# rahulaggarwal965/vslam

Hardware: AMD Instinct MI355X
Metric: frame-pairs/sec (extract+match+RANSAC) @1280×720, 2k kp, 4096 hyp; 1/2/4/8 GPU (higher is better)
Workload: dtype u8/f32/f64; 1 GPU; C3: 1280x720, 2000 keypoints, 4096 hypotheses, batch 256 pairs per GPU, SURVEY 8(d) data: rotation + parallax, sub-pixel resampling, 40-45 % outlier matches; pairs_per_gpu=256, batches_in_flight=4

## Files before the change

### vslam_amd/csrc/ransac_count.hip

```cpp
#include "ransac_residual.h"

namespace {
using namespace vs_ransac;

constexpr int kCntHyps = 128;
constexpr int kCntWaves = 8;
constexpr int kCntQueue = 320;
constexpr int kCntLdsMatches = 4096;
constexpr int kScreenMatches = 128;
constexpr int kScreenHyps = 128;
constexpr int kRankThreads = 512;
constexpr int kPilotHyps = kRankThreads / 64;
constexpr int kCandMax = 8;
constexpr float kCntTinyDD = 0x1p-120f;
constexpr int kFcmpOGT = 2, kFcmpOLT = 4, kFcmpULT = 12;
constexpr int kCntRec = 12;
typedef __attribute__((address_space(3))) volatile uint32_t cnt_queue_t;
static_assert(VSLAM_MAX_KP <= 65536, "queue words keep the match index in 16 bits");

__host__ __device__ constexpr int cnt_pad(int n) { return (n + 255) & ~255; }

struct CntBand {
    float lo, hi;
    double beta;
    bool ok;
};
__device__ __forceinline__ CntBand cnt_band(const float *f, float C1, float C2, float threshold) {
    CntBand B;
    bool ok = threshold >= 0x1p-20f && threshold <= 0x1p20f && C1 <= 0x1p20f && C2 <= 0x1p20f;
#pragma unroll
    for (int k = 0; k < 9; k++) ok = ok && fabsf(f[k]) <= 1024.f;
    const double S = ((double)fabsf(f[0]) + (double)fabsf(f[3]) + (double)fabsf(f[1]) + (double)fabsf(f[4])) * (double)C2 +
                     (double)fabsf(f[6]) + (double)fabsf(f[7]);
    const double beta = 4.04 * 0x1p-24 * S + 1e-30;
    const double sq = sqrt((double)threshold);
    const double lo_r = sq * (1.0 - 0x1p-20) - 1.01 * beta;
    const double hi_r = sq * (1.0 + 0x1p-20) + 2.5 * beta;
    B.lo = lo_r > 0 ? (float)(lo_r * lo_r * (1.0 - 0x1p-22)) : -1.f;
    B.hi = (float)(hi_r * hi_r * (1.0 + 0x1p-20) * (1.0 + 0x1p-22));
    if (!ok) {
        B.lo = -1.f;
        B.hi = INFINITY;
    }
    B.beta = beta;
    B.ok = ok;
    return B;
}
__device__ __forceinline__ void cnt_store_record(float *d, const float *f, const CntBand &B) {
#pragma unroll
    for (int k = 0; k < 9; k++) d[k] = f[k];
    d[9] = B.lo;
    d[10] = B.hi;
    d[11] = B.ok ? (float)(B.beta * (1.0 + 0x1p-20)) : -1.f;
}

struct CntRec {
    float f[9];
    float lo, hi;
    float beta;
};
__device__ __forceinline__ void cnt_load_record(CntRec &R, const float *s_rec, int hh) {
    const float4 *r4 = reinterpret_cast<const float4 *>(s_rec + hh * kCntRec);
    const float4 v0 = r4[0], v1 = r4[1], v2 = r4[2];
    const float f[9] = {v0.x, v0.y, v0.z, v0.w, v1.x, v1.y, v1.z, v1.w, v2.x};
#pragma unroll
    for (int k = 0; k < 9; k++) R.f[k] = f[k];
    R.lo = v2.y;
    R.hi = v2.z;
    R.beta = v2.w;
}

__device__ __forceinline__ v2f cnt_splat(float f) {
    v2f r;
    r.x = f;
    r.y = f;
    return r;
}
__device__ __forceinline__ v2f cnt_cheap(const CntRec &R, const v2f X1, const v2f Y1, const v2f X2, const v2f Y2, v2f &dd) {
    const v2f f0 = cnt_splat(R.f[0]), f1 = cnt_splat(R.f[1]), f2 = cnt_splat(R.f[2]), f3 = cnt_splat(R.f[3]), f4 = cnt_splat(R.f[4]),
              f5 = cnt_splat(R.f[5]), f6 = cnt_splat(R.f[6]), f7 = cnt_splat(R.f[7]), f8 = cnt_splat(R.f[8]);
    const v2f a0 = (f0 * X1 + f1 * Y1) + f2;
    const v2f a1 = (f3 * X1 + f4 * Y1) + f5;
    const v2f a2 = (f6 * X1 + f7 * Y1) + f8;
    const v2f n = (X2 * a0 + Y2 * a1) + a2;
    const v2f nn = n * n;
    dd = a0 * a0;
    v2f r;
    r.x = __builtin_amdgcn_rcpf(dd.x);
    r.y = __builtin_amdgcn_rcpf(dd.y);
    v2f g = __builtin_elementwise_fma(a1, a1, nn * r);
    const v2f t0 = __builtin_elementwise_fma(f3, Y2, __builtin_elementwise_fma(f0, X2, f6));
    const v2f t1 = __builtin_elementwise_fma(f4, Y2, __builtin_elementwise_fma(f1, X2, f7));
    g = __builtin_elementwise_fma(t0, t0, g);
    g = __builtin_elementwise_fma(t1, t1, g);
    return g;
}

__device__ __forceinline__ void cnt_drain(const cnt_queue_t *q, int from, int count, int lane, const float *s_rec,
                                          int *s_cnt, const float *cx1, const float *cy1, const float *cx2, const float *cy2,
                                          float threshold) {
    if (lane < count) {
        const uint32_t en = q[from + lane];
        const int hh = (int)(en >> 16), i = (int)(en & 0xFFFFu);
        ResidualF R;
#pragma unroll
        for (int k = 0; k < 9; k++) R.f[k] = s_rec[hh * kCntRec + k];
        residual_prepare(R);
        const float x2 = cx2[i], y2 = cy2[i];
        const float e = residual_e(R, make_float4(cx1[i], cy1[i], x2, y2), (double)x2, (double)y2);
        if (e <= threshold) atomicAdd(&s_cnt[hh], 1);
    }
}

__device__ __forceinline__ void cnt_push(cnt_queue_t *q, int &qn, unsigned long long U, int hh, int idx, int lane) {
    const int rank = (int)__builtin_amdgcn_mbcnt_hi((uint32_t)(U >> 32), __builtin_amdgcn_mbcnt_lo((uint32_t)U, 0u));
    if ((U >> lane) & 1ull) q[qn + rank] = ((uint32_t)hh << 16) | (uint32_t)idx;
    qn += __popcll(U);
}

template <bool PARTIAL>
__device__ __forceinline__ void cnt_eval_pair(const CntRec &R, const v2f X1, const v2f Y1, const v2f X2, const v2f Y2, int ix,
                                              int m, int &cnt, unsigned long long &ua, unsigned long long &ub,
                                              float &ddmin, v2f &acc) {
    v2f dd;
    v2f g = cnt_cheap(R, X1, Y1, X2, Y2, dd);
    ddmin = fminf(ddmin, fminf(dd.x, dd.y));
    unsigned long long ia = __builtin_amdgcn_fcmpf(g.x, R.lo, kFcmpOLT), oa = __builtin_amdgcn_fcmpf(g.x, R.hi, kFcmpOGT);
    unsigned long long ib = __builtin_amdgcn_fcmpf(g.y, R.lo, kFcmpOLT), ob = __builtin_amdgcn_fcmpf(g.y, R.hi, kFcmpOGT);
    if (PARTIAL) {
        const bool in_a = ix < m, in_b = ix + 1 < m;
        const unsigned long long va = __ballot(in_a), vb = __ballot(in_b);
        ia &= va;
        ib &= vb;
        ua = va & ~(ia | oa);
        ub = vb & ~(ib | ob);
        g.x = in_a ? g.x : 0.f;
        g.y = in_b ? g.y : 0.f;
    } else {
        ua = ~(ia | oa);
        ub = ~(ib | ob);
    }
    cnt += __popcll(ia) + __popcll(ib);
    acc += g;
}

__device__ __forceinline__ float wave_sum_to_lane63(float v) {
    const int z = 0;
    v += __int_as_float(__builtin_amdgcn_update_dpp(z, __float_as_int(v), 0xB1, 0xF, 0xF, false));
    v += __int_as_float(__builtin_amdgcn_update_dpp(z, __float_as_int(v), 0x4E, 0xF, 0xF, false));
    v += __int_as_float(__builtin_amdgcn_update_dpp(z, __float_as_int(v), 0x141, 0xF, 0xF, false));
    v += __int_as_float(__builtin_amdgcn_update_dpp(z, __float_as_int(v), 0x140, 0xF, 0xF, false));
    v += __int_as_float(__builtin_amdgcn_update_dpp(z, __float_as_int(v), 0x142, 0xA, 0xF, false));
    v += __int_as_float(__builtin_amdgcn_update_dpp(z, __float_as_int(v), 0x143, 0xC, 0xF, false));
    return v;
}

template <bool PARTIAL>
__device__ __forceinline__ void cnt_sub_block(const CntRec &R, const float4 X1, const float4 Y1, const float4 X2, const float4 Y2,
                                              int ix, int hh, int lane, int m, int &cnt, cnt_queue_t *q, int &qn, v2f &acc,
                                              int *s_unk, int &pot, bool &unk) {
    unsigned long long u0, u1, u2, u3;
    int c = 0;
    float ddmin = INFINITY;
    v2f x1a, y1a, x2a, y2a, x1b, y1b, x2b, y2b;
    x1a.x = X1.x; x1a.y = X1.y; x1b.x = X1.z; x1b.y = X1.w;
    y1a.x = Y1.x; y1a.y = Y1.y; y1b.x = Y1.z; y1b.y = Y1.w;
    x2a.x = X2.x; x2a.y = X2.y; x2b.x = X2.z; x2b.y = X2.w;
    y2a.x = Y2.x; y2a.y = Y2.y; y2b.x = Y2.z; y2b.y = Y2.w;
    cnt_eval_pair<PARTIAL>(R, x1a, y1a, x2a, y2a, ix, m, c, u0, u1, ddmin, acc);
    cnt_eval_pair<PARTIAL>(R, x1b, y1b, x2b, y2b, ix + 2, m, c, u2, u3, ddmin, acc);
    if (__builtin_amdgcn_fcmpf(ddmin, kCntTinyDD, kFcmpULT) != 0ull) {
        if (lane == 0) s_unk[hh] = 1;
        unk = true;
        c = 0;
        u0 = __builtin_amdgcn_sicmp(ix, m, 40);
        u1 = __builtin_amdgcn_sicmp(ix + 1, m, 40);
        u2 = __builtin_amdgcn_sicmp(ix + 2, m, 40);
        u3 = __builtin_amdgcn_sicmp(ix + 3, m, 40);
    }
    cnt += c;
    pot += c;
    if ((u0 | u1 | u2 | u3) != 0ull) {
        pot += __popcll(u0) + __popcll(u1) + __popcll(u2) + __popcll(u3);
        if (u0) cnt_push(q, qn, u0, hh, ix, lane);
        if (u1) cnt_push(q, qn, u1, hh, ix + 1, lane);
        if (u2) cnt_push(q, qn, u2, hh, ix + 2, lane);
        if (u3) cnt_push(q, qn, u3, hh, ix + 3, lane);
    }
}

__device__ __forceinline__ int cnt_exact_ranked(const float *F9, const float *r, int kp_pad, int m, float threshold, int lane,
                                                double *sum_out = nullptr) {
    ResidualF R;
#pragma unroll
    for (int j = 0; j < 9; j++) R.f[j] = F9[j];
    residual_prepare(R);
    int count = 0;
    double esum = 0;
    for (int i0 = 0; i0 < m; i0 += 256) {
        float4 c[4];
#pragma unroll
        for (int u = 0; u < 4; u++) {
            const int i = i0 + u * 64 + lane;
            c[u] = make_float4(r[i], r[kp_pad + i], r[2 * kp_pad + i], r[3 * kp_pad + i]);
        }
#pragma unroll
        for (int u = 0; u < 4; u++) {
            const float e = residual_e(R, c[u], (double)c[u].z, (double)c[u].w);
            count += __popcll(__ballot(i0 + u * 64 + lane < m && e <= threshold));
            if (sum_out && i0 + u * 64 + lane < m) esum += (double)e;
        }
    }
    if (sum_out) {
#pragma unroll
        for (int off = 32; off > 0; off >>= 1) esum += __shfl_xor(esum, off, 64);
        *sum_out = esum;
    }
    return count;
}

__global__ __launch_bounds__(kRankThreads) void ransac_rank_kernel(
    const float *__restrict__ xy1, const float *__restrict__ xy2, const int32_t *__restrict__ pairs,
    const int32_t *__restrict__ m_arr, int min_m, int kp_stride, int kp_pad, int hyp, float threshold,
    const float *__restrict__ hypF, int32_t *__restrict__ cbound, float *__restrict__ rk, float *__restrict__ cmax,
    unsigned long long *__restrict__ sfloor) {
    const int b = blockIdx.x, tid = threadIdx.x, lane = tid & 63;
    const int wave = __builtin_amdgcn_readfirstlane(tid >> 6);
    const int m = min(m_arr[b], kp_stride);
    if (m < min_m) return;
    __shared__ double s_psum[kPilotHyps];
    __shared__ unsigned long long s_bits[kPilotHyps][VSLAM_MAX_KP / 64];
    __shared__ int s_hist[kPilotHyps][kPilotHyps + 1], s_off[kPilotHyps][kPilotHyps + 1], s_pcount[kPilotHyps];
    const float2 *P1 = reinterpret_cast<const float2 *>(xy1) + (size_t)b * kp_stride;
    const float2 *P2 = reinterpret_cast<const float2 *>(xy2) + (size_t)b * kp_stride;
    const int2 *PR = reinterpret_cast<const int2 *>(pairs) + (size_t)b * kp_stride;
    const int npil = min(kPilotHyps, hyp);
    const int G = (m + 63) >> 6;

    if (wave < npil) {
        const int h = (int)(((long long)hyp * wave) / npil);
        ResidualF R;
        const float *src = hypF + ((size_t)b * hyp + h) * 9;
#pragma unroll
        for (int j = 0; j < 9; j++) R.f[j] = src[j];
        residual_prepare(R);
        int count = 0;
        double esum = 0;
        float c1 = 0.f, c2 = 0.f;
        for (int g0 = 0; g0 < G; g0 += 4) {
            int2 pr[4];
            float2 a[4], c[4];
#pragma unroll
            for (int u = 0; u < 4; u++) pr[u] = PR[min((g0 + u) * 64 + lane, m - 1)];
#pragma unroll
            for (int u = 0; u < 4; u++) {
                a[u] = P1[pr[u].x];
                c[u] = P2[pr[u].y];
            }
#pragma unroll
            for (int u = 0; u < 4; u++) {
                const float e = residual_e(R, make_float4(a[u].x, a[u].y, c[u].x, c[u].y), (double)c[u].x, (double)c[u].y);
                const unsigned long long in = __ballot((g0 + u) * 64 + lane < m && e <= threshold);
                count += __popcll(in);
                if ((g0 + u) * 64 + lane < m) esum += (double)e;
                if (lane == 0 && g0 + u < G) s_bits[wave][g0 + u] = in;
                c1 = fmaxf(c1, fmaxf(fabsf(a[u].x), fabsf(a[u].y)));
                c2 = fmaxf(c2, fmaxf(fabsf(c[u].x), fabsf(c[u].y)));
            }
        }
#pragma unroll
        for (int off = 32; off > 0; off >>= 1) esum += __shfl_xor(esum, off, 64);
        if (lane == 0) {
            s_pcount[wave] = count;
            s_psum[wave] = esum;
        }
        if (wave == 0) {
#pragma unroll
            for (int off = 32; off > 0; off >>= 1) {
                c1 = fmaxf(c1, __shfl_xor(c1, off, 64));
                c2 = fmaxf(c2, __shfl_xor(c2, off, 64));
            }
            if (lane == 0) {
                cmax[2 * b] = c1;
                cmax[2 * b + 1] = c2;
            }
        }
    }
    __syncthreads();

    const int gpw = (G + kPilotHyps - 1) / kPilotHyps;
    const int g_lo = min(G, wave * gpw), g_hi = min(G, g_lo + gpw);
    int hist[kPilotHyps + 1];
#pragma unroll
    for (int v = 0; v <= kPilotHyps; v++) hist[v] = 0;
    for (int g = g_lo; g < g_hi; g++) {
        const bool valid = g * 64 + lane < m;
        int key = 0;
        for (int w = 0; w < npil; w++) key += (int)((~s_bits[w][g] >> lane) & 1ull);
#pragma unroll
        for (int v = 0; v <= kPilotHyps; v++) hist[v] += __popcll(__ballot(valid && key == v));
    }
    if (lane == 0) {
#pragma unroll
        for (int v = 0; v <= kPilotHyps; v++) s_hist[wave][v] = hist[v];
    }
    __syncthreads();
    if (tid == 0) {
        int best = 0;
        for (int w = 0; w < npil; w++) best = max(best, s_pcount[w]);
        cbound[b] = best;
        if (sfloor) {
            double fl = -INFINITY;
            bool any_nan = false;
            for (int w = 0; w < npil; w++)
                if (s_pcount[w] == best) {
                    any_nan = any_nan || !(s_psum[w] == s_psum[w]);
                    if (s_psum[w] > fl) fl = s_psum[w];
                }
            const bool valid = best > 0 && !any_nan && fl > 0 && fl < 0x1p120;
            sfloor[b] = valid ? ((unsigned long long)(uint32_t)best << 32) | (unsigned long long)__float_as_uint((float)(fl * (1.0 - 0x1p-20))) : 0ull;
        }
        int run = 0;
        for (int v = kPilotHyps; v >= 0; v--)
            for (int w = 0; w < kPilotHyps; w++) {
                s_off[w][v] = run;
                run += s_hist[w][v];
            }
    }
    __syncthreads();
    int off[kPilotHyps + 1];
#pragma unroll
    for (int v = 0; v <= kPilotHyps; v++) off[v] = s_off[wave][v];
    float *r = rk + (size_t)b * 4 * kp_pad;
    for (int g = g_lo; g < g_hi; g++) {
        const int i = g * 64 + lane;
        const bool valid = i < m;
        int key = 0;
        for (int w = 0; w < npil; w++) key += (int)((~s_bits[w][g] >> lane) & 1ull);
        int pos = 0;
#pragma unroll
        for (int v = 0; v <= kPilotHyps; v++) {
            const unsigned long long bal = __ballot(valid && key == v);
            const int rank = (int)__builtin_amdgcn_mbcnt_hi((uint32_t)(bal >> 32), __builtin_amdgcn_mbcnt_lo((uint32_t)bal, 0u));
            if (key == v) pos = off[v] + rank;
            off[v] += __popcll(bal);
        }
        if (valid) {
            const int2 pr = PR[i];
            const float2 a = P1[pr.x], c = P2[pr.y];
            r[pos] = a.x;
            r[kp_pad + pos] = a.y;
            r[2 * kp_pad + pos] = c.x;
            r[3 * kp_pad + pos] = c.y;
        }
    }
    const int mpad = cnt_pad(m);
    if (m + tid < mpad) {
        const int2 pr = PR[m - 1];
        const float2 a = P1[pr.x], c = P2[pr.y];
        r[m + tid] = a.x;
        r[kp_pad + m + tid] = a.y;
        r[2 * kp_pad + m + tid] = c.x;
        r[3 * kp_pad + m + tid] = c.y;
    }
}

__global__ __launch_bounds__(256) void ransac_screen_kernel(
    const float *__restrict__ rk, int kp_pad, const int32_t *__restrict__ m_arr, int min_m, int kp_stride, int hyp,
    float threshold, const float *__restrict__ hypF, const float *__restrict__ cmax, int32_t *__restrict__ pot0) {
    const int b = blockIdx.y, tid = threadIdx.x, lane = tid & 63;
    const int wave = __builtin_amdgcn_readfirstlane(tid >> 6);
    const int hbase = blockIdx.x * kScreenHyps;
    const int m = min(m_arr[b], kp_stride);
    if (m < min_m) return;
    __shared__ __align__(16) float s_rec[kScreenHyps * kCntRec];
    if (tid < kScreenHyps) {
        const float *src = hypF + ((size_t)b * hyp + min(hbase + tid, hyp - 1)) * 9;
        float f[9];
#pragma unroll
        for (int k = 0; k < 9; k++) f[k] = src[k];
        const CntBand B = cnt_band(f, cmax[2 * b], cmax[2 * b + 1], threshold);
        cnt_store_record(s_rec + tid * kCntRec, f, B);
    }
    const int n0 = min(m, kScreenMatches);
    const float *r = rk + (size_t)b * 4 * kp_pad;
    const float2 x1 = *reinterpret_cast<const float2 *>(r + 2 * lane);
    const float2 y1 = *reinterpret_cast<const float2 *>(r + kp_pad + 2 * lane);
    const float2 x2 = *reinterpret_cast<const float2 *>(r + 2 * kp_pad + 2 * lane);
    const float2 y2 = *reinterpret_cast<const float2 *>(r + 3 * kp_pad + 2 * lane);
    v2f X1, Y1, X2, Y2;
    X1.x = x1.x; X1.y = x1.y; Y1.x = y1.x; Y1.y = y1.y;
    X2.x = x2.x; X2.y = x2.y; Y2.x = y2.x; Y2.y = y2.y;
    const unsigned long long va = __ballot(2 * lane < n0), vb = __ballot(2 * lane + 1 < n0);
    __syncthreads();
    int mine = 0;
    constexpr int kU = 4;
    for (int j = 0; j < 32; j += kU) {
        CntRec R[kU];
        v2f dd[kU], g[kU];
#pragma unroll
        for (int u = 0; u < kU; u++) cnt_load_record(R[u], s_rec, wave * 32 + j + u);
#pragma unroll
        for (int u = 0; u < kU; u++) g[u] = cnt_cheap(R[u], X1, Y1, X2, Y2, dd[u]);
#pragma unroll
        for (int u = 0; u < kU; u++) {
            const unsigned long long oa = __builtin_amdgcn_fcmpf(g[u].x, R[u].hi, kFcmpOGT), ob = __builtin_amdgcn_fcmpf(g[u].y, R[u].hi, kFcmpOGT);
            int p = __popcll(va & ~oa) + __popcll(vb & ~ob);
            if (__builtin_amdgcn_fcmpf(fminf(dd[u].x, dd[u].y), kCntTinyDD, kFcmpULT) != 0ull) p = n0;
            mine = lane == j + u ? p : mine;
        }
    }
    const int h = hbase + wave * 32 + lane;
    if (lane < 32 && h < hyp) pot0[(size_t)b * hyp + h] = mine;
}

__global__ __launch_bounds__(64 * kCandMax) void ransac_cand_kernel(
    const float *__restrict__ rk, int kp_pad, const int32_t *__restrict__ m_arr, int min_m, int kp_stride, int hyp,
    float threshold, const float *__restrict__ hypF, const int32_t *__restrict__ pot0, int by_sum,
    int32_t *__restrict__ cbound, unsigned long long *__restrict__ sfloor) {
    const int b = blockIdx.x, tid = threadIdx.x, lane = tid & 63;
    const int wave = __builtin_amdgcn_readfirstlane(tid >> 6);
    const int m = min(m_arr[b], kp_stride);
    if (m < min_m) return;
    __shared__ int s_max[kCandMax], s_l0[kCandMax][kCandMax], s_l1[kCandMax][kCandMax], s_n0[kCandMax], s_n1[kCandMax];
    __shared__ int s_cand[kCandMax], s_nc;
    const int32_t *P = pot0 + (size_t)b * hyp;
    int mx = -1;
    for (int i = tid; i < hyp; i += 64 * kCandMax) mx = max(mx, P[i]);
#pragma unroll
    for (int off = 32; off > 0; off >>= 1) mx = max(mx, __shfl_xor(mx, off, 64));
    if (lane == 0) s_max[wave] = mx;
    __syncthreads();
    mx = s_max[0];
    for (int w = 1; w < kCandMax; w++) mx = max(mx, s_max[w]);
    const int per = (hyp + kCandMax - 1) / kCandMax;
    const int lo = min(hyp, wave * per), hi = min(hyp, lo + per);
    int n0 = 0, n1 = 0;
    __shared__ int s_samp[kCandMax][32];
    int nsamp = 0;
    for (int i0 = lo; i0 < hi && ((by_sum && nsamp < 32) || n0 < kCandMax || n1 < kCandMax); i0 += 64) {
        const int i = i0 + lane;
        const int v = i < hi ? P[i] : -2;
        unsigned long long b0 = __ballot(v == mx), b1 = __ballot(v == mx - 1);
        if (by_sum) {
            const int rs = nsamp + __popcll(b0 & ((1ull << lane) - 1ull));
            if (v == mx && rs < 32) s_samp[wave][rs] = i;
            nsamp = min(32, nsamp + (int)__popcll(b0));
        }
        const int r0 = n0 + __popcll(b0 & ((1ull << lane) - 1ull)), r1 = n1 + __popcll(b1 & ((1ull << lane) - 1ull));
        if (v == mx && r0 < kCandMax) s_l0[wave][r0] = i;
        if (v == mx - 1 && r1 < kCandMax) s_l1[wave][r1] = i;
        n0 = min(kCandMax, n0 + __popcll(b0));
        n1 = min(kCandMax, n1 + __popcll(b1));
    }
    if (by_sum && nsamp > 1) {
        const int n128 = min(m, kScreenMatches);
        const float *r = rk + (size_t)b * 4 * kp_pad;
        const float2 x1 = *reinterpret_cast<const float2 *>(r + 2 * lane), y1 = *reinterpret_cast<const float2 *>(r + kp_pad + 2 * lane);
        const float2 x2 = *reinterpret_cast<const float2 *>(r + 2 * kp_pad + 2 * lane), y2 = *reinterpret_cast<const float2 *>(r + 3 * kp_pad + 2 * lane);
        v2f X1, Y1, X2, Y2;
        X1.x = x1.x; X1.y = x1.y; Y1.x = y1.x; Y1.y = y1.y;
        X2.x = x2.x; X2.y = x2.y; Y2.x = y2.x; Y2.y = y2.y;
        float fl[9];
        {
            const int hs = s_samp[wave][lane < nsamp ? lane : 0];
            const float *src = hypF + ((size_t)b * hyp + hs) * 9;
#pragma unroll
            for (int k = 0; k < 9; k++) fl[k] = src[k];
        }
        float best_s = -INFINITY;
        int best_i = -1;
        for (int j = 0; j < nsamp; j++) {
            CntRec R;
#pragma unroll
            for (int k = 0; k < 9; k++) R.f[k] = __int_as_float(__builtin_amdgcn_readlane(__float_as_int(fl[k]), j));
            v2f dd;
            const v2f g = cnt_cheap(R, X1, Y1, X2, Y2, dd);
            const float part = wave_sum_to_lane63((2 * lane < n128 ? g.x : 0.f) + (2 * lane + 1 < n128 ? g.y : 0.f));
            const float tot = __int_as_float(__builtin_amdgcn_readlane(__float_as_int(part), 63));
            if (tot > best_s) {
                best_s = tot;
                best_i = s_samp[wave][j];
            }
        }
        if (lane == 0 && best_i >= 0 && n0 > 0) {
            const int old = s_l0[wave][0];
            for (int k = 1; k < n0; k++)
                if (s_l0[wave][k] == best_i) s_l0[wave][k] = old;
            s_l0[wave][0] = best_i;
        }
    }
    if (lane == 0) {
        s_n0[wave] = n0;
        s_n1[wave] = n1;
    }
    __syncthreads();
    if (tid == 0) {
        int n = 0;
        for (int w = 0; w < kCandMax && n < kCandMax; w++)
            if (s_n0[w] > 0) s_cand[n++] = s_l0[w][0];
        for (int w = 0; w < kCandMax && n < kCandMax; w++)
            for (int k = 1; k < s_n0[w] && n < kCandMax; k++) s_cand[n++] = s_l0[w][k];
        for (int w = 0; w < kCandMax && n < kCandMax; w++)
            for (int k = 0; k < s_n1[w] && n < kCandMax; k++) s_cand[n++] = s_l1[w][k];
        s_nc = n;
    }
    __syncthreads();
    __shared__ int s_ccount[kCandMax];
    __shared__ double s_csum[kCandMax];
    if (wave < s_nc) {
        const int h = s_cand[wave];
        double esum = 0;
        const int count = cnt_exact_ranked(hypF + ((size_t)b * hyp + h) * 9, rk + (size_t)b * 4 * kp_pad, kp_pad, m, threshold, lane, &esum);
        if (lane == 0) {
            atomicMax(&cbound[b], count);
            s_ccount[wave] = count;
            s_csum[wave] = esum;
        }
    }
    __syncthreads();
    if (tid == 0) {
        int cb = -1;
        for (int k = 0; k < s_nc; k++) cb = max(cb, s_ccount[k]);
        double fl = -INFINITY;
        bool any_nan = false;
        for (int k = 0; k < s_nc; k++)
            if (s_ccount[k] == cb) {
                any_nan = any_nan || !(s_csum[k] == s_csum[k]);
                if (s_csum[k] > fl) fl = s_csum[k];
            }
        const bool valid = cb > 0 && !any_nan && fl > 0 && fl < 0x1p120;
        const float flf = (float)(fl * (1.0 - 0x1p-20));
        const unsigned long long mine = valid ? ((unsigned long long)(uint32_t)cb << 32) | (unsigned long long)__float_as_uint(flf) : 0ull;
        const unsigned long long pilots = sfloor[b];
        sfloor[b] = mine > pilots ? mine : pilots;
    }
}

template <bool LDS>
__global__ __launch_bounds__(64 * kCntWaves) __attribute__((amdgpu_waves_per_eu(6, 6))) void ransac_count_kernel(
    const float *__restrict__ rk, int kp_pad, const int32_t *__restrict__ m_arr, int min_m, int kp_stride, int hyp, float threshold,
    const float *__restrict__ hypF, const int32_t *__restrict__ pot0, const float *__restrict__ cmax,
    int32_t *__restrict__ hyp_count, float *__restrict__ hyp_sum, float *__restrict__ approx, int32_t *__restrict__ cbound,
    const unsigned long long *__restrict__ sfloor) {
    const int b = blockIdx.y, tid = threadIdx.x, lane = tid & 63;
    const int wave = __builtin_amdgcn_readfirstlane(tid >> 6);
    const int hbase = blockIdx.x * kCntHyps;
    const int nh = min(kCntHyps, hyp - hbase);
    const int m = min(m_arr[b], kp_stride);
    if (m < min_m) return;

    __shared__ __align__(16) float s_rec[kCntHyps * kCntRec];
    __shared__ int s_cnt[kCntHyps];
    __shared__ float s_part[kCntHyps];
    __shared__ int s_unk[kCntHyps];
    __shared__ int s_state[kCntHyps];
    __shared__ int s_list[kCntHyps];
    constexpr int kListWaves = kCntHyps / 64;
    static_assert(kCntHyps % 64 == 0 && kListWaves <= kCntWaves, "whole waves find the survivors");
    __shared__ int s_nlist[kListWaves], s_next, s_bound;
    extern __shared__ __align__(16) uint32_t s_dyn[];

    const int n0 = min(m, kScreenMatches);
    const int bound0 = cbound[b];
    if (tid < kCntHyps) {
        const bool alive = tid < nh && pot0[(size_t)b * hyp + hbase + tid] + (m - n0) >= bound0;
        s_cnt[tid] = 0;
        s_unk[tid] = 0;
        s_part[tid] = 0.f;
        s_state[tid] = alive ? 1 : 0;
        const unsigned long long bal = __ballot(alive);
        if (alive) s_list[wave * 64 + __popcll(bal & ((1ull << lane) - 1ull))] = tid;
        if (lane == 0) s_nlist[wave] = __popcll(bal);
    }
    if (tid == 0) {
        s_next = 0;
        s_bound = bound0;
    }
    __syncthreads();
    int n_alive = 0;
#pragma unroll
    for (int w = 0; w < kListWaves; w++) n_alive += s_nlist[w];
    const size_t out = (size_t)b * hyp + hbase + tid;
    if (n_alive == 0) {
        if (tid < nh) {
            hyp_count[out] = -1;
            hyp_sum[out] = __int_as_float(0x7FC00000);
            reinterpret_cast<float2 *>(approx)[out] = make_float2(0.f, INFINITY);
        }
        return;
    }

    double my_beta = 0;
    bool my_ok = false;
    if (tid < kCntHyps && s_state[tid]) {
        const float *src = hypF + ((size_t)b * hyp + hbase + tid) * 9;
        float f[9];
#pragma unroll
        for (int k = 0; k < 9; k++) f[k] = src[k];
        const CntBand B = cnt_band(f, cmax[2 * b], cmax[2 * b + 1], threshold);
        my_beta = B.beta;
        my_ok = B.ok;
        cnt_store_record(s_rec + tid * kCntRec, f, B);
    }
    const int mpad = cnt_pad(m);
    const float *rg = rk + (size_t)b * 4 * kp_pad;
    float *s_co = reinterpret_cast<float *>(s_dyn);
    if (LDS) {
        for (int k = tid * 4; k < mpad; k += 64 * kCntWaves * 4) {
#pragma unroll
            for (int a = 0; a < 4; a++)
                *reinterpret_cast<float4 *>(s_co + a * mpad + k) = *reinterpret_cast<const float4 *>(rg + (size_t)a * kp_pad + k);
        }
    }
    __syncthreads();
    const int cstride = LDS ? mpad : kp_pad;
    const float *cx1 = LDS ? s_co : rg;
    const float *cy1 = cx1 + cstride, *cx2 = cx1 + 2 * cstride, *cy2 = cx1 + 3 * cstride;

    {
        cnt_queue_t *q = (cnt_queue_t *)(s_dyn + (LDS ? 4 * mpad : 0) + wave * kCntQueue);
        int qn = 0;
        int bound = bound0;
        const unsigned long long fkey = sfloor ? sfloor[b] : 0ull;
        const int floor_count = fkey != 0ull ? (int)(fkey >> 32) : -1;
        const float floor_sum = __uint_as_float((uint32_t)fkey);
        const int nsub = mpad >> 8;
        const bool part = (m & 255) != 0;
        int k = 0;
        if (lane == 0) k = atomicAdd(&s_next, 1);
        k = __builtin_amdgcn_readfirstlane(k);
        while (k < n_alive) {
            int knext = 0;
            if (lane == 0) knext = atomicAdd(&s_next, 1);
            int hh;
            {
                int kk = k, w = 0;
                while (w + 1 < kListWaves && kk >= s_nlist[w]) kk -= s_nlist[w++];
                hh = s_list[w * 64 + kk];
            }
            bound = max(bound, *(__attribute__((address_space(3))) const volatile int *)&s_bound);
            CntRec R;
            cnt_load_record(R, s_rec, hh);
            int cnt = 0, pot = 0, seen = 0;
            bool dropped = false, unk = false;
            v2f acc;
            acc.x = 0.f;
            acc.y = 0.f;
            for (int s = 0; s < nsub; s++) {
                const int ix = s * 256 + 4 * lane;
                const float4 X1 = *reinterpret_cast<const float4 *>(cx1 + ix), Y1 = *reinterpret_cast<const float4 *>(cy1 + ix);
                const float4 X2 = *reinterpret_cast<const float4 *>(cx2 + ix), Y2 = *reinterpret_cast<const float4 *>(cy2 + ix);
                if (s == nsub - 1 && part) {
                    cnt_sub_block<true>(R, X1, Y1, X2, Y2, ix, hh, lane, m, cnt, q, qn, acc, s_unk, pot, unk);
                    seen += m & 255;
                } else {
                    cnt_sub_block<false>(R, X1, Y1, X2, Y2, ix, hh, lane, m, cnt, q, qn, acc, s_unk, pot, unk);
                    seen += 256;
                }
                while (qn >= 64) {
                    cnt_drain(q, qn - 64, 64, lane, s_rec, s_cnt, cx1, cy1, cx2, cy2, threshold);
                    qn -= 64;
                }
                if (pot + (m - seen) < bound) {
                    dropped = true;
                    break;
                }
                if (seen < m && bound == floor_count && pot + (m - seen) == bound && !unk && R.beta >= 0.f) {
                    const float S = __int_as_float(__builtin_amdgcn_readlane(__float_as_int(wave_sum_to_lane63(acc.x + acc.y)), 63));
                    const float ns = (float)seen;
                    const float err = (2.02f * R.beta * sqrtf(ns * S) + ns * R.beta * R.beta + 0x1p-18f * S) * 1.0001f;
                    const float upper = ((S + err) + threshold * (float)(m - seen)) * 1.0001f;
                    if (upper < floor_sum * 0.9999f) {
                        dropped = true;
                        break;
                    }
                }
            }
            if (dropped) {
                if (lane == 0) s_state[hh] = 2;
            } else {
                const float part_sum = wave_sum_to_lane63(acc.x + acc.y);
                if (lane == 63) s_part[hh] = part_sum;
                if (lane == 0) {
                    if (cnt) atomicAdd(&s_cnt[hh], cnt);
                    if (cnt > bound) {
                        atomicMax(&s_bound, cnt);
                        atomicMax(&cbound[b], cnt);
                    }
                }
                bound = max(bound, cnt);
            }
            k = __builtin_amdgcn_readfirstlane(knext);
        }
        if (qn > 0) cnt_drain(q, 0, qn, lane, s_rec, s_cnt, cx1, cy1, cx2, cy2, threshold);
    }
    __syncthreads();
    if (tid < nh) {
        const int st = s_state[tid];
        hyp_count[out] = st == 1 ? s_cnt[tid] : -1;
        hyp_sum[out] = __int_as_float(0x7FC00000);
        const float S = s_part[tid];
        float err = INFINITY;
        if (st == 1 && my_ok && !s_unk[tid]) {
            const double Sd = (double)S;
            err = (float)((2.02 * my_beta * sqrt((double)m * Sd) + (double)m * my_beta * my_beta + 0x1p-18 * Sd) * (1.0 + 0x1p-20));
        }
        reinterpret_cast<float2 *>(approx)[out] = make_float2(S, err);
    }
}

}

int vs_launch_ransac_count(vslam_ctx *ctx, const float *xy1, const float *xy2, const int32_t *pairs, const int32_t *m,
                           const float *hypF, int batch, int kp_stride, int hyp, float threshold, int32_t *hyp_count,
                           float *hyp_sum, float *approx) {
    const int min_m = ctx->ransac_min_matches;
    int rc;
    int32_t *cbound = nullptr, *pot0 = nullptr;
    float *rk = nullptr, *cmax = nullptr;
    const int kp_pad = cnt_pad(kp_stride);
    if ((rc = vs_arena_get(ctx, "ransac.cbound", sizeof(int32_t) * (size_t)batch, (void **)&cbound))) return rc;
    unsigned long long *sfloor = nullptr;
    if ((rc = vs_arena_get(ctx, "ransac.sfloor", sizeof(unsigned long long) * (size_t)batch, (void **)&sfloor))) return rc;
    static const bool no_sum_rule = VS_EXPERIMENT_ENV("VSLAM_RANSAC_NO_SUM_RULE") != nullptr;
    const unsigned long long *use_floor = no_sum_rule ? nullptr : sfloor;
    if ((rc = vs_arena_get(ctx, "ransac.pot0", sizeof(int32_t) * (size_t)batch * hyp, (void **)&pot0))) return rc;
    if ((rc = vs_arena_get(ctx, "ransac.rk", sizeof(float) * 4 * (size_t)kp_pad * batch, (void **)&rk))) return rc;
    if ((rc = vs_arena_get(ctx, "ransac.cmax", sizeof(float) * 2 * (size_t)batch, (void **)&cmax))) return rc;
    {
        VsProfScope ps(ctx, "ransac_rank_kernel");
        ransac_rank_kernel<<<batch, kRankThreads, 0, ctx->stream>>>(xy1, xy2, pairs, m, min_m, kp_stride, kp_pad, hyp, threshold, hypF,
                                                                    cbound, rk, cmax, sfloor);
    }
    {
        VsProfScope ps(ctx, "ransac_screen_kernel");
        dim3 grid(vs_div_up(hyp, kScreenHyps), batch);
        ransac_screen_kernel<<<grid, 256, 0, ctx->stream>>>(rk, kp_pad, m, min_m, kp_stride, hyp, threshold, hypF, cmax, pot0);
    }
    {
        VsProfScope ps(ctx, "ransac_cand_kernel");
        ransac_cand_kernel<<<batch, 64 * kCandMax, 0, ctx->stream>>>(rk, kp_pad, m, min_m, kp_stride, hyp, threshold, hypF, pot0,
                                                                     no_sum_rule ? 0 : 1, cbound, sfloor);
    }
    if (int arc = vs_aux_job_point(ctx, 4)) return arc;
    {
        VsProfScope ps(ctx, "ransac_count_kernel");
        const bool lds = kp_pad <= kCntLdsMatches;
        const size_t dyn = (lds ? sizeof(float) * 4 * (size_t)kp_pad : 0) + sizeof(uint32_t) * kCntQueue * kCntWaves;
        if (dyn > 32 * 1024 &&
            (rc = vs_allow_dynamic_lds(ctx, ransac_count_kernel<true>, "ransac_count",
                                       sizeof(float) * 4 * kCntLdsMatches + sizeof(uint32_t) * kCntQueue * kCntWaves)))
            return rc;
        dim3 grid(vs_div_up(hyp, kCntHyps), batch);
        if (lds)
            ransac_count_kernel<true><<<grid, 64 * kCntWaves, dyn, ctx->stream>>>(rk, kp_pad, m, min_m, kp_stride, hyp, threshold, hypF, pot0,
                                                                                  cmax, hyp_count, hyp_sum, approx, cbound, use_floor);
        else
            ransac_count_kernel<false><<<grid, 64 * kCntWaves, dyn, ctx->stream>>>(rk, kp_pad, m, min_m, kp_stride, hyp, threshold, hypF, pot0,
                                                                                   cmax, hyp_count, hyp_sum, approx, cbound, use_floor);
    }
    return VSLAM_OK;
}
```

Before: 93780 frame-pairs/s.

## Reuse screen-kernel head counts and sums so count kernel skips first 128 matches

```diff
diff --git a/vslam_amd/csrc/ransac_count.hip b/vslam_amd/csrc/ransac_count.hip
--- a/vslam_amd/csrc/ransac_count.hip
+++ b/vslam_amd/csrc/ransac_count.hip
@@ -19,6 +19,8 @@
 static_assert(VSLAM_MAX_KP <= 65536, "queue words keep the match index in 16 bits");
 
 __host__ __device__ constexpr int cnt_pad(int n) { return (n + 255) & ~255; }
+constexpr int kHeadUncertified = -1;
+__device__ __forceinline__ float cnt_sum_rel(int adds) { return fmaxf(0x1p-18f, (float)(13 + adds) * 0x1p-24f); }
 
 struct CntBand {
     float lo, hi;
@@ -367,7 +369,8 @@
 
 __global__ __launch_bounds__(256) void ransac_screen_kernel(
     const float *__restrict__ rk, int kp_pad, const int32_t *__restrict__ m_arr, int min_m, int kp_stride, int hyp,
-    float threshold, const float *__restrict__ hypF, const float *__restrict__ cmax, int32_t *__restrict__ pot0) {
+    float threshold, const float *__restrict__ hypF, const float *__restrict__ cmax, const int32_t *__restrict__ cbound,
+    int32_t *__restrict__ pot0, int2 *__restrict__ head) {
     const int b = blockIdx.y, tid = threadIdx.x, lane = tid & 63;
     const int wave = __builtin_amdgcn_readfirstlane(tid >> 6);
     const int hbase = blockIdx.x * kScreenHyps;
@@ -383,6 +386,7 @@
         cnt_store_record(s_rec + tid * kCntRec, f, B);
     }
     const int n0 = min(m, kScreenMatches);
+    const int bound_pilots = cbound[b];
     const float *r = rk + (size_t)b * 4 * kp_pad;
     const float2 x1 = *reinterpret_cast<const float2 *>(r + 2 * lane);
     const float2 y1 = *reinterpret_cast<const float2 *>(r + kp_pad + 2 * lane);
@@ -394,7 +398,11 @@
     const unsigned long long va = __ballot(2 * lane < n0), vb = __ballot(2 * lane + 1 < n0);
     __syncthreads();
     int mine = 0;
+    float mine_sum = 0.f;
+    const bool odd1 = (lane & 1) != 0, odd2 = (lane & 2) != 0;
+    const bool in_a = 2 * lane < n0, in_b = 2 * lane + 1 < n0;
     constexpr int kU = 4;
+    static_assert(kU == 4, "the head sums are reduced four hypotheses at a time");
     for (int j = 0; j < 32; j += kU) {
         CntRec R[kU];
         v2f dd[kU], g[kU];
@@ -402,16 +410,42 @@
         for (int u = 0; u < kU; u++) cnt_load_record(R[u], s_rec, wave * 32 + j + u);
 #pragma unroll
         for (int u = 0; u < kU; u++) g[u] = cnt_cheap(R[u], X1, Y1, X2, Y2, dd[u]);
+        bool any_alive = false;
 #pragma unroll
         for (int u = 0; u < kU; u++) {
             const unsigned long long oa = __builtin_amdgcn_fcmpf(g[u].x, R[u].hi, kFcmpOGT), ob = __builtin_amdgcn_fcmpf(g[u].y, R[u].hi, kFcmpOGT);
+            const unsigned long long ia = __builtin_amdgcn_fcmpf(g[u].x, R[u].lo, kFcmpOLT), ib = __builtin_amdgcn_fcmpf(g[u].y, R[u].lo, kFcmpOLT);
             int p = __popcll(va & ~oa) + __popcll(vb & ~ob);
-            if (__builtin_amdgcn_fcmpf(fminf(dd[u].x, dd[u].y), kCntTinyDD, kFcmpULT) != 0ull) p = n0;
-            mine = lane == j + u ? p : mine;
-        }
+            int c = __popcll(va & ia) + __popcll(vb & ib);
+            if (__builtin_amdgcn_fcmpf(fminf(dd[u].x, dd[u].y), kCntTinyDD, kFcmpULT) != 0ull) {
+                p = n0;
+                c = 0xFF;
+            }
+            mine = lane == j + u ? (p | (c << 8)) : mine;
+            any_alive = any_alive || p + (m - n0) >= bound_pilots;
+        }
+        if (!any_alive) continue;
+        float v[kU];
+#pragma unroll
+        for (int u = 0; u < kU; u++) v[u] = (in_a ? g[u].x : 0.f) + (in_b ? g[u].y : 0.f);
+        const int z = 0;
+        const float k01 = odd1 ? v[1] : v[0], t01 = odd1 ? v[0] : v[1], k23 = odd1 ? v[3] : v[2], t23 = odd1 ? v[2] : v[3];
+        const float r01 = k01 + __int_as_float(__builtin_amdgcn_update_dpp(z, __float_as_int(t01), 0xB1, 0xF, 0xF, false));
+        const float r23 = k23 + __int_as_float(__builtin_amdgcn_update_dpp(z, __float_as_int(t23), 0xB1, 0xF, 0xF, false));
+        const float kk = odd2 ? r23 : r01, tt = odd2 ? r01 : r23;
+        float r = kk + __int_as_float(__builtin_amdgcn_update_dpp(z, __float_as_int(tt), 0x4E, 0xF, 0xF, false));
+        r += __int_as_float(__builtin_amdgcn_update_dpp(z, __float_as_int(r), 0x124, 0xF, 0xF, false));
+        r += __int_as_float(__builtin_amdgcn_update_dpp(z, __float_as_int(r), 0x128, 0xF, 0xF, false));
+        r += __shfl_xor(r, 16, 64);
+        r += __shfl_xor(r, 32, 64);
+        mine_sum = (lane >> 2) == (j >> 2) ? r : mine_sum;
     }
     const int h = hbase + wave * 32 + lane;
-    if (lane < 32 && h < hyp) pot0[(size_t)b * hyp + h] = mine;
+    if (lane < 32 && h < hyp) {
+        const int c = mine >> 8;
+        pot0[(size_t)b * hyp + h] = mine & 0xFF;
+        head[(size_t)b * hyp + h] = make_int2(c == 0xFF ? kHeadUncertified : c, __float_as_int(mine_sum));
+    }
 }
 
 __global__ __launch_bounds__(64 * kCandMax) void ransac_cand_kernel(
@@ -537,12 +571,19 @@
     }
 }
 
-template <bool LDS>
+#ifdef VSLAM_EXPERIMENTS
+#define VS_CNT_PAYLOAD_PARAM , int exit_payload
+#define VS_CNT_PAYLOAD_ARG , exit_payload
+#else
+#define VS_CNT_PAYLOAD_PARAM
+#define VS_CNT_PAYLOAD_ARG
+#endif
+template <bool LDS, bool ZERO>
 __global__ __launch_bounds__(64 * kCntWaves) __attribute__((amdgpu_waves_per_eu(6, 6))) void ransac_count_kernel(
     const float *__restrict__ rk, int kp_pad, const int32_t *__restrict__ m_arr, int min_m, int kp_stride, int hyp, float threshold,
-    const float *__restrict__ hypF, const int32_t *__restrict__ pot0, const float *__restrict__ cmax,
-    int32_t *__restrict__ hyp_count, float *__restrict__ hyp_sum, float *__restrict__ approx, int32_t *__restrict__ cbound,
-    const unsigned long long *__restrict__ sfloor) {
+    const float *__restrict__ hypF, const int32_t *__restrict__ pot0, const int2 *__restrict__ head,
+    const float *__restrict__ cmax, int32_t *__restrict__ hyp_count, float *__restrict__ hyp_sum, float *__restrict__ approx,
+    int32_t *__restrict__ cbound, const unsigned long long *__restrict__ sfloor VS_CNT_PAYLOAD_PARAM) {
     const int b = blockIdx.y, tid = threadIdx.x, lane = tid & 63;
     const int wave = __builtin_amdgcn_readfirstlane(tid >> 6);
     const int hbase = blockIdx.x * kCntHyps;
@@ -553,6 +594,7 @@
     __shared__ __align__(16) float s_rec[kCntHyps * kCntRec];
     __shared__ int s_cnt[kCntHyps];
     __shared__ float s_part[kCntHyps];
+    constexpr int kHeadMine = 0x10000, kHeadNoSum = 0x20000;
     __shared__ int s_unk[kCntHyps];
     __shared__ int s_state[kCntHyps];
     __shared__ int s_list[kCntHyps];
@@ -564,11 +606,21 @@
     const int n0 = min(m, kScreenMatches);
     const int bound0 = cbound[b];
     if (tid < kCntHyps) {
-        const bool alive = tid < nh && pot0[(size_t)b * hyp + hbase + tid] + (m - n0) >= bound0;
-        s_cnt[tid] = 0;
+        const int p0 = tid < nh ? pot0[(size_t)b * hyp + hbase + tid] : 0;
+        const bool alive = tid < nh && p0 + (m - n0) >= bound0;
+        int certain = 0, word = p0;
+        float hsum = 0.f;
+        if (!ZERO && alive) {
+            const int2 hd = head[(size_t)b * hyp + hbase + tid];
+            if (hd.x == p0) certain = hd.x;
+            else word |= kHeadMine;
+            if (hd.x != kHeadUncertified) hsum = __int_as_float(hd.y);
+            else word |= kHeadNoSum;
+        }
+        s_cnt[tid] = certain;
         s_unk[tid] = 0;
-        s_part[tid] = 0.f;
-        s_state[tid] = alive ? 1 : 0;
+        s_part[tid] = hsum;
+        s_state[tid] = (alive ? 1 : 0) | (ZERO ? 0 : word << 2);
         const unsigned long long bal = __ballot(alive);
         if (alive) s_list[wave * 64 + __popcll(bal & ((1ull << lane) - 1ull))] = tid;
         if (lane == 0) s_nlist[wave] = __popcll(bal);
@@ -593,7 +645,7 @@
 
     double my_beta = 0;
     bool my_ok = false;
-    if (tid < kCntHyps && s_state[tid]) {
+    if (tid < kCntHyps && (s_state[tid] & 3)) {
         const float *src = hypF + ((size_t)b * hyp + hbase + tid) * 9;
         float f[9];
 #pragma unroll
@@ -625,8 +677,10 @@
         const unsigned long long fkey = sfloor ? sfloor[b] : 0ull;
         const int floor_count = fkey != 0ull ? (int)(fkey >> 32) : -1;
         const float floor_sum = __uint_as_float((uint32_t)fkey);
-        const int nsub = mpad >> 8;
-        const bool part = (m & 255) != 0;
+        const int org = ZERO ? 0 : n0;
+        const int nsub = (m - org + 255) >> 8;
+        const bool part = ((m - org) & 255) != 0;
+        const float sum_rel = cnt_sum_rel(2 * nsub + 9);
         int k = 0;
         if (lane == 0) k = atomicAdd(&s_next, 1);
         k = __builtin_amdgcn_readfirstlane(k);
@@ -642,18 +696,25 @@
             bound = max(bound, *(__attribute__((address_space(3))) const volatile int *)&s_bound);
             CntRec R;
             cnt_load_record(R, s_rec, hh);
-            int cnt = 0, pot = 0, seen = 0;
+            const int word = ZERO ? 0 : s_state[hh] >> 2;
+            const int head_cnt = ZERO ? 0 : *(__attribute__((address_space(3))) const volatile int *)&s_cnt[hh];
+            float head_sum = ZERO ? 0.f : s_part[hh];
+            int cnt = 0, pot = word & 0xFFFF, seen = org;
             bool dropped = false, unk = false;
             v2f acc;
             acc.x = 0.f;
             acc.y = 0.f;
-            for (int s = 0; s < nsub; s++) {
-                const int ix = s * 256 + 4 * lane;
-                const float4 X1 = *reinterpret_cast<const float4 *>(cx1 + ix), Y1 = *reinterpret_cast<const float4 *>(cy1 + ix);
-                const float4 X2 = *reinterpret_cast<const float4 *>(cx2 + ix), Y2 = *reinterpret_cast<const float4 *>(cy2 + ix);
-                if (s == nsub - 1 && part) {
-                    cnt_sub_block<true>(R, X1, Y1, X2, Y2, ix, hh, lane, m, cnt, q, qn, acc, s_unk, pot, unk);
-                    seen += m & 255;
+            for (int s = 0;; s++) {
+                if (s >= nsub && (ZERO || s > nsub || !(word & kHeadMine))) break;
+                const bool hd = !ZERO && s == nsub;
+                const int pot_walk = pot;
+                const int ix = (hd ? 0 : org + s * 256) + 4 * lane;
+                const int il = min(ix, mpad - 4);
+                const float4 X1 = *reinterpret_cast<const float4 *>(cx1 + il), Y1 = *reinterpret_cast<const float4 *>(cy1 + il);
+                const float4 X2 = *reinterpret_cast<const float4 *>(cx2 + il), Y2 = *reinterpret_cast<const float4 *>(cy2 + il);
+                if (hd || (s == nsub - 1 && part)) {
+                    cnt_sub_block<true>(R, X1, Y1, X2, Y2, ix, hh, lane, hd ? n0 : m, cnt, q, qn, acc, s_unk, pot, unk);
+                    seen += hd ? 0 : (m - org) & 255;
                 } else {
                     cnt_sub_block<false>(R, X1, Y1, X2, Y2, ix, hh, lane, m, cnt, q, qn, acc, s_unk, pot, unk);
                     seen += 256;
@@ -662,14 +723,19 @@
                     cnt_drain(q, qn - 64, 64, lane, s_rec, s_cnt, cx1, cy1, cx2, cy2, threshold);
                     qn -= 64;
                 }
+                if (hd) {
+                    head_sum = 0.f;
+                    pot = pot_walk;
+                    break;
+                }
                 if (pot + (m - seen) < bound) {
                     dropped = true;
                     break;
                 }
-                if (seen < m && bound == floor_count && pot + (m - seen) == bound && !unk && R.beta >= 0.f) {
-                    const float S = __int_as_float(__builtin_amdgcn_readlane(__float_as_int(wave_sum_to_lane63(acc.x + acc.y)), 63));
+                if (seen < m && bound == floor_count && pot + (m - seen) == bound && !unk && R.beta >= 0.f && !(word & kHeadNoSum)) {
+                    const float S = head_sum + __int_as_float(__builtin_amdgcn_readlane(__float_as_int(wave_sum_to_lane63(acc.x + acc.y)), 63));
                     const float ns = (float)seen;
-                    const float err = (2.02f * R.beta * sqrtf(ns * S) + ns * R.beta * R.beta + 0x1p-18f * S) * 1.0001f;
+                    const float err = (2.02f * R.beta * sqrtf(ns * S) + ns * R.beta * R.beta + sum_rel * S) * 1.0001f;
                     const float upper = ((S + err) + threshold * (float)(m - seen)) * 1.0001f;
                     if (upper < floor_sum * 0.9999f) {
                         dropped = true;
@@ -678,18 +744,36 @@
                 }
             }
             if (dropped) {
+#ifdef VSLAM_EXPERIMENTS
+                if (lane == 0) s_state[hh] = 2 | (seen << 2);
+#else
                 if (lane == 0) s_state[hh] = 2;
+#endif
             } else {
-                const float part_sum = wave_sum_to_lane63(acc.x + acc.y);
+                const float part_sum = head_sum + wave_sum_to_lane63(acc.x + acc.y);
+                bool beaten = false;
+                if (bound == floor_count && pot == bound && !unk && R.beta >= 0.f) {
+                    const float S = __int_as_float(__builtin_amdgcn_readlane(__float_as_int(part_sum), 63));
+                    const float ns = (float)m;
+                    const float err = (2.02f * R.beta * sqrtf(ns * S) + ns * R.beta * R.beta + sum_rel * S) * 1.0001f;
+                    beaten = (S + err) * 1.0001f < floor_sum * 0.9999f;
+                }
                 if (lane == 63) s_part[hh] = part_sum;
-                if (lane == 0) {
+                const int certain = head_cnt + cnt;
+                if (beaten) {
+#ifdef VSLAM_EXPERIMENTS
+                    if (lane == 0) s_state[hh] = 2 | (seen << 2);
+#else
+                    if (lane == 0) s_state[hh] = 2;
+#endif
+                } else if (lane == 0) {
                     if (cnt) atomicAdd(&s_cnt[hh], cnt);
-                    if (cnt > bound) {
-                        atomicMax(&s_bound, cnt);
-                        atomicMax(&cbound[b], cnt);
+                    if (certain > bound) {
+                        atomicMax(&s_bound, certain);
+                        atomicMax(&cbound[b], certain);
                     }
                 }
-                bound = max(bound, cnt);
+                if (!beaten) bound = max(bound, certain);
             }
             k = __builtin_amdgcn_readfirstlane(knext);
         }
@@ -697,14 +781,19 @@
     }
     __syncthreads();
     if (tid < nh) {
-        const int st = s_state[tid];
+        const int st = s_state[tid] & 3;
         hyp_count[out] = st == 1 ? s_cnt[tid] : -1;
-        hyp_sum[out] = __int_as_float(0x7FC00000);
-        const float S = s_part[tid];
+        int nan_bits = 0x7FC00000;
+#ifdef VSLAM_EXPERIMENTS
+        if (exit_payload && st != 1) nan_bits |= st == 2 ? min(s_state[tid] >> 2, 0x3FFFFF) : 0x3FFFFF;
+#endif
+        hyp_sum[out] = __int_as_float(nan_bits);
+        const float S = st == 1 ? s_part[tid] : 0.f;
         float err = INFINITY;
         if (st == 1 && my_ok && !s_unk[tid]) {
             const double Sd = (double)S;
-            err = (float)((2.02 * my_beta * sqrt((double)m * Sd) + (double)m * my_beta * my_beta + 0x1p-18 * Sd) * (1.0 + 0x1p-20));
+            const double rel = (double)cnt_sum_rel(2 * ((m - (ZERO ? 0 : n0) + 255) >> 8) + 9);
+            err = (float)((2.02 * my_beta * sqrt((double)m * Sd) + (double)m * my_beta * my_beta + rel * Sd) * (1.0 + 0x1p-20));
         }
         reinterpret_cast<float2 *>(approx)[out] = make_float2(S, err);
     }
@@ -724,6 +813,12 @@
     unsigned long long *sfloor = nullptr;
     if ((rc = vs_arena_get(ctx, "ransac.sfloor", sizeof(unsigned long long) * (size_t)batch, (void **)&sfloor))) return rc;
     static const bool no_sum_rule = VS_EXPERIMENT_ENV("VSLAM_RANSAC_NO_SUM_RULE") != nullptr;
+    const bool from_zero = VS_EXPERIMENT_ENV("VSLAM_RANSAC_COUNT_FROM_ZERO") != nullptr;
+#ifdef VSLAM_EXPERIMENTS
+    const int exit_payload = VS_EXPERIMENT_ENV("VSLAM_RANSAC_COUNT_EXIT_PAYLOAD") != nullptr ? 1 : 0;
+#endif
+    int2 *head = nullptr;
+    if ((rc = vs_arena_get(ctx, "ransac.head", sizeof(int2) * (size_t)batch * hyp, (void **)&head))) return rc;
     const unsigned long long *use_floor = no_sum_rule ? nullptr : sfloor;
     if ((rc = vs_arena_get(ctx, "ransac.pot0", sizeof(int32_t) * (size_t)batch * hyp, (void **)&pot0))) return rc;
     if ((rc = vs_arena_get(ctx, "ransac.rk", sizeof(float) * 4 * (size_t)kp_pad * batch, (void **)&rk))) return rc;
@@ -736,7 +831,7 @@
     {
         VsProfScope ps(ctx, "ransac_screen_kernel");
         dim3 grid(vs_div_up(hyp, kScreenHyps), batch);
-        ransac_screen_kernel<<<grid, 256, 0, ctx->stream>>>(rk, kp_pad, m, min_m, kp_stride, hyp, threshold, hypF, cmax, pot0);
+        ransac_screen_kernel<<<grid, 256, 0, ctx->stream>>>(rk, kp_pad, m, min_m, kp_stride, hyp, threshold, hypF, cmax, cbound, pot0, head);
     }
     {
         VsProfScope ps(ctx, "ransac_cand_kernel");
@@ -748,17 +843,35 @@
         VsProfScope ps(ctx, "ransac_count_kernel");
         const bool lds = kp_pad <= kCntLdsMatches;
         const size_t dyn = (lds ? sizeof(float) * 4 * (size_t)kp_pad : 0) + sizeof(uint32_t) * kCntQueue * kCntWaves;
+        const size_t dyn_max = sizeof(float) * 4 * kCntLdsMatches + sizeof(uint32_t) * kCntQueue * kCntWaves;
+        dim3 grid(vs_div_up(hyp, kCntHyps), batch);
+#ifdef VSLAM_EXPERIMENTS
+        if (from_zero) {
+            if (dyn > 32 * 1024 && (rc = vs_allow_dynamic_lds(ctx, ransac_count_kernel<true, true>, "ransac_count_from_zero", dyn_max)))
+                return rc;
+            if (lds)
+                ransac_count_kernel<true, true><<<grid, 64 * kCntWaves, dyn, ctx->stream>>>(
+                    rk, kp_pad, m, min_m, kp_stride, hyp, threshold, hypF, pot0, head, cmax, hyp_count, hyp_sum, approx, cbound,
+                    use_floor VS_CNT_PAYLOAD_ARG);
+            else
+                ransac_count_kernel<false, true><<<grid, 64 * kCntWaves, dyn, ctx->stream>>>(
+                    rk, kp_pad, m, min_m, kp_stride, hyp, threshold, hypF, pot0, head, cmax, hyp_count, hyp_sum, approx, cbound,
+                    use_floor VS_CNT_PAYLOAD_ARG);
+            return VSLAM_OK;
+        }
+#endif
+        (void)from_zero;
         if (dyn > 32 * 1024 &&
-            (rc = vs_allow_dynamic_lds(ctx, ransac_count_kernel<true>, "ransac_count",
-                                       sizeof(float) * 4 * kCntLdsMatches + sizeof(uint32_t) * kCntQueue * kCntWaves)))
+            (rc = vs_allow_dynamic_lds(ctx, ransac_count_kernel<true, false>, "ransac_count", dyn_max)))
             return rc;
-        dim3 grid(vs_div_up(hyp, kCntHyps), batch);
         if (lds)
-            ransac_count_kernel<true><<<grid, 64 * kCntWaves, dyn, ctx->stream>>>(rk, kp_pad, m, min_m, kp_stride, hyp, threshold, hypF, pot0,
-                                                                                  cmax, hyp_count, hyp_sum, approx, cbound, use_floor);
+            ransac_count_kernel<true, false><<<grid, 64 * kCntWaves, dyn, ctx->stream>>>(
+                rk, kp_pad, m, min_m, kp_stride, hyp, threshold, hypF, pot0, head, cmax, hyp_count, hyp_sum, approx, cbound,
+                    use_floor VS_CNT_PAYLOAD_ARG);
         else
-            ransac_count_kernel<false><<<grid, 64 * kCntWaves, dyn, ctx->stream>>>(rk, kp_pad, m, min_m, kp_stride, hyp, threshold, hypF, pot0,
-                                                                                   cmax, hyp_count, hyp_sum, approx, cbound, use_floor);
+            ransac_count_kernel<false, false><<<grid, 64 * kCntWaves, dyn, ctx->stream>>>(
+                rk, kp_pad, m, min_m, kp_stride, hyp, threshold, hypF, pot0, head, cmax, hyp_count, hyp_sum, approx, cbound,
+                    use_floor VS_CNT_PAYLOAD_ARG);
     }
     return VSLAM_OK;
 }
```

Result: faster. 96060 frame-pairs/s (median of 6 runs) (+2.4%).
